# Ugness/MeBT

Measured on AMD Instinct MI355X. Metric: masked video tokens/sec/GPU (train step, 24L d=1024, 1024+256 tok), higher is better.
Workload: dtype bf16; 1 GPU; Sky-Timelapse 16f MeBT train step: 24L/1024d/16h, 1024 VQ tokens + 256 latents, batch 6/GPU, t=0.5 (NC=NT=512), fwd + masked CE + bwd + AdamW; global_batch=6, parallelism=dp1, optimizer=in-backward (fused into the weight-gradient launches)

## Files before the change

### include/mebt_hip.h

```cpp
#ifndef MEBT_HIP_H
#define MEBT_HIP_H

#include <stdint.h>

#ifdef __cplusplus
extern "C" {
#endif

#define MEBT_ABI_VERSION 2
#define MEBT_MAX_LAYERS 128

typedef void* mebt_stream_t;
typedef struct mebt_model mebt_model;

enum mebt_status { MEBT_STATUS_OK = 0, MEBT_STATUS_EINVAL = 1, MEBT_STATUS_ESHAPE = 2, MEBT_STATUS_EHIP = 3,
                   MEBT_STATUS_EWORKSPACE = 4, MEBT_STATUS_EDTYPE = 5 };
enum mebt_dtype { MEBT_DTYPE_F32 = 0, MEBT_DTYPE_BF16 = 1, MEBT_DTYPE_F16 = 2  };
enum mebt_mode { MEBT_MODE_LATENT_ENC = 0, MEBT_MODE_LATENT_SELF = 1, MEBT_MODE_LATENT_DEC = 2, MEBT_MODE_LT2L = 3,
                 MEBT_MODE_MASKGIT = 4  };

typedef struct mebt_model_desc {
    int32_t n_layer, n_head, n_embd, vocab, n_latent , block_size;
    int32_t dtype;
    int32_t modes[MEBT_MAX_LAYERS];
// ... 146 lines not shown
int mebt_op_i3d_head(int32_t dtype, const void* x, const float* w, const float* bias, float* pooled, float* logits, int32_t B, int32_t T,
                     int32_t H, int32_t W, int32_t C, int32_t ncls, mebt_stream_t stream);

int mebt_profile_enable(int32_t on);
int mebt_profile_read(int32_t family, double* launches, double* total_ms, double* total_flops);
int64_t mebt_profile_dump(char* buf, int64_t cap);
int32_t mebt_profile_read_waits(int32_t cap, int32_t* layer, double* ms);
int mebt_debug_dropout_mask(uint64_t seed, uint32_t site, float p, int64_t n, float* out, mebt_stream_t stream);
int mebt_debug_clock_probe(unsigned long long* out4, uint64_t ref_ticks_100mhz, mebt_stream_t stream);
void mebt_debug_side_stream(mebt_model* m, int32_t on);
void mebt_debug_set_side_stream(mebt_model* m, mebt_stream_t stream);
void mebt_debug_gemm_tile(int32_t bm, int32_t bn);
void mebt_debug_gemm_variant(int32_t dma);
void mebt_debug_gemm_scratch(void* buf, int64_t bytes);
void mebt_debug_gemm_stamps(unsigned long long* buf);
void mebt_debug_grouped_config(int32_t tbm, int32_t tbn, int32_t ring);
void mebt_debug_grouped_stages(int32_t n);

#ifdef __cplusplus
}
#endif
#endif
```

### mebt_amd/_lib.py

```python
import ctypes as C
import os

_HERE = os.path.dirname(os.path.abspath(__file__))
LIB_PATH = os.environ.get("MEBT_HIP_LIB") or os.path.join(_HERE, "lib", "libmebt_hip.so")

SHIPPED_TUNE = os.path.join(_HERE, "tune", "gfx950.txt")

MEBT_MAX_LAYERS = 128
F32, BF16, F16 = 0, 1, 2
EPI_NONE, EPI_GELU, EPI_RESID, EPI_GELU_BWD = 0, 1, 2, 3
MODE_IDS = {"latent_enc": 0, "latent_self": 1, "latent_dec": 2, "lt2l": 3, "maskgit": 4}

c_i32, c_i64, c_f32, c_vp = C.c_int32, C.c_int64, C.c_float, C.c_void_p


class ModelDesc(C.Structure):
    _fields_ = [("n_layer", c_i32), ("n_head", c_i32), ("n_embd", c_i32), ("vocab", c_i32),
                ("n_latent", c_i32), ("block_size", c_i32), ("dtype", c_i32),
                ("modes", c_i32 * MEBT_MAX_LAYERS), ("label_smoothing", c_f32),
                ("embd_pdrop", c_f32), ("resid_pdrop", c_f32), ("attn_pdrop", c_f32)]


PROTOTYPES = {
    "mebt_last_error": (C.c_char_p, []),
# ... 48 lines not shown
    "mebt_op_cast_f16": (c_i32, [c_vp, c_vp, c_i64, c_vp]),
    "mebt_op_i3d_preprocess": (c_i32, [c_i32, c_vp, c_vp, c_i32, c_i32, c_i32, c_i32, c_i32, c_vp]),
    "mebt_op_i3d_conv": (c_i32, [c_i32, c_vp, c_vp]),
    "mebt_op_i3d_maxpool": (c_i32, [c_i32, c_vp, c_vp] + [c_i32] * 11 + [c_vp]),
    "mebt_op_i3d_head": (c_i32, [c_i32, c_vp, c_vp, c_vp, c_vp, c_vp] + [c_i32] * 6 + [c_vp]),
    "mebt_debug_dropout_mask": (c_i32, [C.c_uint64, C.c_uint32, c_f32, c_i64, c_vp, c_vp]),
    "mebt_debug_clock_probe": (c_i32, [c_vp, C.c_uint64, c_vp]),
    "mebt_debug_side_stream": (None, [c_vp, c_i32]),
    "mebt_debug_set_side_stream": (None, [c_vp, c_vp]),
    "mebt_debug_gemm_tile": (None, [c_i32, c_i32]),
    "mebt_debug_gemm_variant": (None, [c_i32]),
    "mebt_debug_grouped_stages": (None, [c_i32]),
    "mebt_debug_gemm_scratch": (None, [c_vp, c_i64]),
    "mebt_debug_gemm_stamps": (None, [c_vp]),
    "mebt_debug_grouped_config": (None, [c_i32, c_i32, c_i32]),
    "mebt_gemm_autotune": (None, [c_i32]),
    "mebt_gemm_autotune_enabled": (c_i32, []),
    "mebt_gemm_tune_export": (c_i64, [C.c_char_p, c_i64]),
    "mebt_gemm_tune_import": (c_i32, [C.c_char_p, c_i32]),
    "mebt_gemm_tune_alternatives": (c_i64, [C.c_char_p, c_i64]),
    "mebt_profile_enable": (c_i32, [c_i32]),
    "mebt_profile_read": (c_i32, [c_i32, C.POINTER(C.c_double), C.POINTER(C.c_double), C.POINTER(C.c_double)]),
    "mebt_profile_dump": (c_i64, [C.c_char_p, c_i64]),
    "mebt_profile_read_waits": (c_i32, [c_i32, C.POINTER(C.c_int32), C.POINTER(C.c_double)]),
}

_lib = None


def load():
# ... 53 lines not shown
```

### mebt_amd/csrc/attention.hip

```cpp
#include "common.h"
#include "kernels.h"

namespace {

constexpr int KT = 32;

template <typename T, int HD>
__device__ __forceinline__ void load_row(const T* src, float (&dst)[HD], float scale = 1.f) {
#pragma unroll
    for (int e = 0; e < HD; e += 4) {
        const f32x4 v = load4<T>(src + e);
        dst[e] = v[0] * scale; dst[e + 1] = v[1] * scale; dst[e + 2] = v[2] * scale; dst[e + 3] = v[3] * scale;
    }
}
template <typename T, int HD>
__device__ __forceinline__ void store_row(T* dst, const float (&src)[HD], float scale = 1.f) {
#pragma unroll
    for (int e = 0; e < HD; e += 4) store4<T>(dst + e, f32x4{src[e] * scale, src[e + 1] * scale, src[e + 2] * scale, src[e + 3] * scale});
}

template <typename T, int HD>
__device__ __forceinline__ void stage_tile(float (*dst)[HD], const T* src, int ld, int n, int tid, int nthreads) {
    constexpr int CPR = HD / 4;
    for (int c = tid; c < KT * CPR; c += nthreads) {
// ... 261 lines not shown
        const dim3 gk((p.NK + 63) / 64, p.H, p.B);
        if (NS > 1 && !one && p.NQ >= NS * KT) hipLaunchKernelGGL((attn_bwd_dkv_generic<T, HD, NS>), gk, dim3(64 * NS), (attn_lds_bytes<HD, NS>()), stream, p);
        else hipLaunchKernelGGL((attn_bwd_dkv_generic<T, HD, 1>), gk, dim3(64), (attn_lds_bytes<HD, 1>()), stream, p);
    }
    return MEBT_OK;
}

}

#ifdef MEBT_HAVE_ATTN_MFMA
int launch_attn_fwd_mfma(const AttnParams& p, hipStream_t stream);
int launch_attn_bwd_mfma(const AttnParams& p, hipStream_t stream);
#else
static int launch_attn_fwd_mfma(const AttnParams&, hipStream_t) { return -1; }
static int launch_attn_bwd_mfma(const AttnParams&, hipStream_t) { return -1; }
#endif
#ifdef MEBT_HAVE_ATTN_MFMA
static int g_force_generic = 0;
#else
static int g_force_generic = 1;
#endif
#ifdef MEBT_HAVE_ATTN_MFMA
void mebt_attn_force_generic(int on) { g_force_generic = on; }
#else
void mebt_attn_force_generic(int) {}
#endif

#define DISPATCH_HD(FN, T)                                             \
    switch (p.HD) {                                                    \
        case 32: FN<T, 32>(p, stream); break;                          \
        case 64: FN<T, 64>(p, stream); break;                          \
        case 128: FN<T, 128>(p, stream); break;                        \
        default: mebt_set_error("attention: head size must be 32, 64 or 128"); return MEBT_ESHAPE; \
    }

bool attn_fwd_can_gather(int dtype, int HD) { return dtype == MEBT_BF16 && HD == 64 && !g_force_generic; }

int launch_attn_fwd(const AttnParams& p, int dtype, hipStream_t stream) {
    if (p.B <= 0 || p.NQ <= 0) return MEBT_OK;
    if (dtype == MEBT_BF16 && p.HD == 64 && !g_force_generic && p.NK > 0) return launch_attn_fwd_mfma(p, stream);
    if (p.kidx && p.NK > 0) { mebt_set_error("attention: gathered keys / values (kidx) need the MFMA forward (bf16, head size 64)"); return MEBT_ESHAPE; }
    if (dtype == MEBT_BF16) { DISPATCH_HD(run_fwd, bf16_t) } else { DISPATCH_HD(run_fwd, float) }
// ... 12 lines not shown
```

### mebt_amd/csrc/attention_mfma.hip

```cpp
#include "common.h"
#include "kernels.h"
#include <cstdlib>

namespace {

typedef __attribute__((address_space(3))) s16x4* lds_s16x4_ptr;
typedef short s16x8 __attribute__((ext_vector_type(8)));

constexpr int TILE = 64;
constexpr int TILE_BYTES = TILE * 64 * 2;
constexpr float LOG2E = 1.4426950408889634f;

__device__ __forceinline__ int swz(int row) { return ((row >> 1) & 3) << 1; }

__device__ __forceinline__ bf16x8 frag_rows(const char* tile, int blk16, int ks, int lane) {
    const int row = blk16 * 16 + (lane & 15);
    const int c = 4 * ks + (lane >> 4);
    return *reinterpret_cast<const bf16x8*>(tile + row * 128 + ((c ^ swz(row)) << 4));
}
__device__ __forceinline__ bf16x8 frag_cols(const char* tile, int cb, int kk, int lane) {
    const int g = lane >> 4, i = lane & 15, q4 = i >> 2, pp = i & 3;
    const int ch = 2 * cb + (pp >> 1);
    const int r0 = 32 * kk + 4 * g + q4, r1 = r0 + 16;
    const s16x4 lo = __builtin_amdgcn_ds_read_tr16_b64_v4i16((lds_s16x4_ptr)(tile + r0 * 128 + ((ch ^ swz(r0)) << 4) + 8 * (pp & 1)));
// ... 46 lines not shown
}
typedef unsigned u32x2_t __attribute__((ext_vector_type(2)));
__device__ __forceinline__ float group_sum(float v) {
    u32x2_t r = __builtin_amdgcn_permlane16_swap(__float_as_uint(v), __float_as_uint(v), false, false);
    v = __uint_as_float(r[0]) + __uint_as_float(r[1]);
    r = __builtin_amdgcn_permlane32_swap(__float_as_uint(v), __float_as_uint(v), false, false);
    return __uint_as_float(r[0]) + __uint_as_float(r[1]);
}
__device__ __forceinline__ float group_max(float v) {
    u32x2_t r = __builtin_amdgcn_permlane16_swap(__float_as_uint(v), __float_as_uint(v), false, false);
    v = fmaxf(__uint_as_float(r[0]), __uint_as_float(r[1]));
    r = __builtin_amdgcn_permlane32_swap(__float_as_uint(v), __float_as_uint(v), false, false);
    return fmaxf(__uint_as_float(r[0]), __uint_as_float(r[1]));
}
#define MFMA(a, b, c) __builtin_amdgcn_mfma_f32_16x16x32_bf16(a, b, c, 0, 0, 0)

constexpr int WAVES = 8;
constexpr int BLOCK_ROWS = WAVES * 16;
constexpr int CHUNK_TILES = 4;
constexpr int CHUNK = CHUNK_TILES * TILE;
constexpr int CHUNK_BYTES = CHUNK_TILES * TILE_BYTES;
constexpr int STAT_BYTES = CHUNK * 4;
constexpr int MASK_BYTES = 4096;
constexpr int MASK_OFF = 2 * CHUNK_BYTES + 2 * STAT_BYTES;
constexpr int STAGE_BYTES = MASK_OFF + MASK_BYTES;
constexpr int ATTN_LDS = 2 * STAGE_BYTES;
constexpr int DMA_PER_WAVE = 2 * (CHUNK_BYTES / 1024) / WAVES;

template <int NW = WAVES>
struct ChunkDma {
// ... 26 lines not shown
            const uint32_t off = src[i] >= 0 ? ((uint32_t)src[i] * ld + 8 * (slot ^ swz(row))) * 2 : (uint32_t)MEBT_OOB;
            dma16(rsrc, lds_addr_of(dst + (wave + NW * i) * 1024), off);
        }
    }
};
template <int N> __device__ __forceinline__ void wait_vm() { asm volatile("s_waitcnt vmcnt(%0)" ::"n"(N) : "memory"); }

template <int NW, int NST, int SPLIT = 1>
__global__ __launch_bounds__(NW * SPLIT * 64) void attn_fwd_mfma(const AttnParams p) {
    extern __shared__ __attribute__((aligned(16))) char smem_all[];
    constexpr int CT = NW / 2, CROWS = CT * TILE, CBYTES = CT * TILE_BYTES, SBYTES = 2 * CBYTES;
    const int tid = threadIdx.x, lane = tid & 63, g = lane >> 4;
    const int wave_all = __builtin_amdgcn_readfirstlane(tid >> 6);
    const int half = SPLIT == 1 ? 0 : wave_all / NW, wave = SPLIT == 1 ? wave_all : wave_all % NW;
    char* smem = smem_all + half * (NST * SBYTES);
    const int b = blockIdx.z, h = blockIdx.y;
    const int q = blockIdx.x * (NW * 16) + wave * 16 + (lane & 15);
    const bf16_t* Q = reinterpret_cast<const bf16_t*>(p.q) + (size_t)b * p.NQ * p.ldq + h * 64;
    const bool gather = p.kidx != nullptr;
    const int krows = gather ? p.kidx_rows : p.NK;
    const bf16_t* K = reinterpret_cast<const bf16_t*>(p.k) + (size_t)b * krows * p.ldk + h * 64;
    const bf16_t* V = reinterpret_cast<const bf16_t*>(p.v) + (size_t)b * krows * p.ldv + h * 64;
    bf16x8 qf[2];
#pragma unroll
    for (int ks = 0; ks < 2; ++ks) qf[ks] = frag_global(Q, q, p.NQ, p.ldq, ks, lane);
    ChunkDma<NW> lk, lv;
    lk.init(K, krows, p.ldk, wave, lane);
    lv.init(V, krows, p.ldv, wave, lane);
    int* sidx = reinterpret_cast<int*>(smem_all + SPLIT * NST * SBYTES);
    if (gather) {
        const int32_t* gi = p.kidx + (size_t)b * p.NK;
        for (int i = tid; i < p.NK; i += NW * SPLIT * 64) sidx[i] = gi[i];
// ... 148 lines not shown
        const float inv = 1.0f / l;
        bf16_t* O = reinterpret_cast<bf16_t*>(p.o) + ((size_t)b * p.NQ + q) * p.ldo + h * 64;
#pragma unroll
        for (int e = 0; e < 4; ++e) store4<bf16_t>(O + 16 * e + 4 * g, o[e] * inv);
        if (p.lse && g == 0) p.lse[((size_t)b * p.H + h) * p.NQ + q] = m * 0.6931471805599453f + logf(l);
    }
}

__global__ __launch_bounds__(512) void attn_fwd_pp(const AttnParams p) {
    extern __shared__ __attribute__((aligned(16))) char smem_all[];
    constexpr int NW = 4, CROWS = 2 * TILE, CBYTES = 2 * TILE_BYTES, SBYTES = 2 * CBYTES;
    const int tid = threadIdx.x, lane = tid & 63, g = lane >> 4;
    const int wave_all = __builtin_amdgcn_readfirstlane(tid >> 6);
    const int half = wave_all >> 2, wave = wave_all & 3;
    char* smem = smem_all + half * (2 * SBYTES);
    const int b = blockIdx.z, h = blockIdx.y;
    const int q = blockIdx.x * (NW * 16) + wave * 16 + (lane & 15);
    const bf16_t* Q = reinterpret_cast<const bf16_t*>(p.q) + (size_t)b * p.NQ * p.ldq + h * 64;
    const bool gather = p.kidx != nullptr;
    const int krows = gather ? p.kidx_rows : p.NK;
    const bf16_t* K = reinterpret_cast<const bf16_t*>(p.k) + (size_t)b * krows * p.ldk + h * 64;
    const bf16_t* V = reinterpret_cast<const bf16_t*>(p.v) + (size_t)b * krows * p.ldv + h * 64;
    bf16x8 qf[2];
#pragma unroll
    for (int ks = 0; ks < 2; ++ks) qf[ks] = frag_global(Q, q, p.NQ, p.ldq, ks, lane);
    ChunkDma<NW> lk, lv;
    lk.init(K, krows, p.ldk, wave, lane);
    lv.init(V, krows, p.ldv, wave, lane);
    int* sidx = reinterpret_cast<int*>(smem_all + 4 * SBYTES);
    if (gather) {
        const int32_t* gi = p.kidx + (size_t)b * p.NK;
        for (int i = tid; i < p.NK; i += 512) sidx[i] = gi[i];
// ... 154 lines not shown
#pragma unroll
        for (int e = 0; e < 4; ++e)
#pragma unroll
            for (int rr = 0; rr < 4; ++rr) o[e][rr] = o[e][rr] * a0 + mg[4 * e + rr] * a1;
        m = mn;
    }
    if (q < p.NQ) {
        const float inv = 1.0f / l;
        bf16_t* O = reinterpret_cast<bf16_t*>(p.o) + ((size_t)b * p.NQ + q) * p.ldo + h * 64;
#pragma unroll
        for (int e = 0; e < 4; ++e) store4<bf16_t>(O + 16 * e + 4 * g, o[e] * inv);
        if (p.lse && g == 0) p.lse[((size_t)b * p.H + h) * p.NQ + q] = m * 0.6931471805599453f + logf(l);
    }
}

__global__ __launch_bounds__(WAVES * 64) void attn_bwd_dq_mfma(const AttnParams p) {
    extern __shared__ __attribute__((aligned(16))) char smem[];
    const int tid = threadIdx.x, lane = tid & 63, g = lane >> 4;
    const int wave = __builtin_amdgcn_readfirstlane(tid >> 6);
    const int b = blockIdx.z, h = blockIdx.y;
    const int q = blockIdx.x * BLOCK_ROWS + wave * 16 + (lane & 15);
    const bool qv = q < p.NQ;
    const bf16_t* Q = reinterpret_cast<const bf16_t*>(p.q) + (size_t)b * p.NQ * p.ldq + h * 64;
    const bf16_t* G = reinterpret_cast<const bf16_t*>(p.d_o) + (size_t)b * p.NQ * p.lddo + h * 64;
    const bf16_t* Oo = reinterpret_cast<const bf16_t*>(p.o) + (size_t)b * p.NQ * p.ldo + h * 64;
    const bf16_t* K = reinterpret_cast<const bf16_t*>(p.k) + (size_t)b * p.NK * p.ldk + h * 64;
    const bf16_t* V = reinterpret_cast<const bf16_t*>(p.v) + (size_t)b * p.NK * p.ldv + h * 64;
    ChunkDma<> lk, lv;
    lk.init(K, p.NK, p.ldk, wave, lane);
    lv.init(V, p.NK, p.ldv, wave, lane);
    const int nchunks = (p.NK + CHUNK - 1) / CHUNK;
    bf16x8 qf[2], gf[2], of[2];
#pragma unroll
    for (int ks = 0; ks < 2; ++ks) {
        qf[ks] = frag_global(Q, q, p.NQ, p.ldq, ks, lane);
        gf[ks] = frag_global(G, q, p.NQ, p.lddo, ks, lane);
        of[ks] = frag_global(Oo, q, p.NQ, p.ldo, ks, lane);
    }
    const size_t sidx = ((size_t)b * p.H + h) * p.NQ + q;
    const float lse_q = qv ? p.lse[sidx] : 0.f;
    const bool use_bits = p.drop.thresh && p.dmask != nullptr;
    const int mtiles = mebt_attn_dmask_tiles(p.NK);
    const size_t mrow0 = ((size_t)b * p.H + h) * p.NQ;
    const __amdgpu_buffer_rsrc_t rmask = make_rsrc(p.dmask ? p.dmask + mrow0 * mtiles * 4 : (const uint16_t*)p.q, use_bits ? (size_t)p.NQ * mtiles * 8 : 0);
    const uint32_t moff = (uint32_t)((blockIdx.x * BLOCK_ROWS + 32 * (wave & 3) + (lane >> 1)) * mtiles * 8 + (lane & 1) * 16);
    auto issue_mask = [&](char* stage, int chunk) {
        if (wave < 4) dma16(rmask, lds_addr_of(stage + MASK_OFF + wave * 1024), moff + (uint32_t)chunk * 32);
    };
    lk.issue(smem, 0, wave);
    lv.issue(smem + CHUNK_BYTES, 0, wave);
    issue_mask(smem, 0);
    if (nchunks > 1) {
        lk.issue(smem + STAGE_BYTES, 1, wave);
        lv.issue(smem + STAGE_BYTES + CHUNK_BYTES, 1, wave);
        issue_mask(smem + STAGE_BYTES, 1);
    }
    float delta = 0.f;
#pragma unroll
    for (int ks = 0; ks < 2; ++ks)
#pragma unroll
        for (int j = 0; j < 8; ++j) delta += (float)gf[ks][j] * (float)of[ks][j];
    delta = group_sum(delta);
    const float lse2 = lse_q * LOG2E;
    const float c = 0.125f * LOG2E;
    FragOffsets fo;
    fo.init(lane);

    f32x4 dq[4];
#pragma unroll
    for (int e = 0; e < 4; ++e) dq[e] = f32x4{0, 0, 0, 0};
    const uint64_t drow = (((uint64_t)b * p.H + h) * p.NQ + q) * p.NK;
    const int mlds = (wave * 16 + (lane & 15)) * 32 + g * 2;
    for (int ch = 0; ch < nchunks; ++ch) {
        char* stage = smem + (ch & 1) * STAGE_BYTES;
        if (ch + 1 < nchunks) { if (wave < 4) wait_vm<DMA_PER_WAVE + 1>(); else wait_vm<DMA_PER_WAVE>(); } else wait_vm<0>();
        __builtin_amdgcn_s_barrier();
        const int nt = min(CHUNK_TILES, (p.NK - ch * CHUNK + TILE - 1) / TILE);
// ... 40 lines not shown
        if (ch + 2 < nchunks) {
            __builtin_amdgcn_s_barrier();
            lk.issue(stage, ch + 2, wave);
            lv.issue(stage + CHUNK_BYTES, ch + 2, wave);
            issue_mask(stage, ch + 2);
        }
    }
    if (qv) {
        bf16_t* D = reinterpret_cast<bf16_t*>(p.dq) + ((size_t)b * p.NQ + q) * p.lddq + h * 64;
#pragma unroll
        for (int e = 0; e < 4; ++e) store4<bf16_t>(D + 16 * e + 4 * g, dq[e]);
        if (g == 0) p.delta[sidx] = delta;
    }
}

__global__ __launch_bounds__(WAVES * 64) void attn_bwd_dkv_mfma(const AttnParams p) {
    extern __shared__ __attribute__((aligned(16))) char smem[];
    const int tid = threadIdx.x, lane = tid & 63, g = lane >> 4;
    const int wave = __builtin_amdgcn_readfirstlane(tid >> 6);
    const int b = blockIdx.z, h = blockIdx.y;
    const int key = blockIdx.x * BLOCK_ROWS + wave * 16 + (lane & 15);
    const bf16_t* Q = reinterpret_cast<const bf16_t*>(p.q) + (size_t)b * p.NQ * p.ldq + h * 64;
    const bf16_t* G = reinterpret_cast<const bf16_t*>(p.d_o) + (size_t)b * p.NQ * p.lddo + h * 64;
    const bf16_t* K = reinterpret_cast<const bf16_t*>(p.k) + (size_t)b * p.NK * p.ldk + h * 64;
    const bf16_t* V = reinterpret_cast<const bf16_t*>(p.v) + (size_t)b * p.NK * p.ldv + h * 64;
    const float* L = p.lse + ((size_t)b * p.H + h) * p.NQ;
    const float* Dl = p.delta + ((size_t)b * p.H + h) * p.NQ;
    ChunkDma<> lq, lg;
    lq.init(Q, p.NQ, p.ldq, wave, lane);
    lg.init(G, p.NQ, p.lddo, wave, lane);
    const __amdgpu_buffer_rsrc_t rstat = make_rsrc(wave == 0 ? L : Dl, (size_t)p.NQ * 4);
    const int nchunks = (p.NQ + CHUNK - 1) / CHUNK;
    const bool use_bits = p.drop.thresh && p.dmask != nullptr;
    const int mtiles = mebt_attn_dmask_tiles(p.NK);
    const size_t mrow0 = ((size_t)b * p.H + h) * p.NQ;
    const __amdgpu_buffer_rsrc_t rmask = make_rsrc(p.dmask ? p.dmask + mrow0 * mtiles * 4 : (const uint16_t*)p.q, use_bits ? (size_t)p.NQ * mtiles * 8 : 0);
    const uint32_t moff = (uint32_t)((64 * (wave & 3) + lane) * mtiles * 8 + blockIdx.x * 16);
    auto issue = [&](char* stage, int chunk) {
        lq.issue(stage, chunk, wave);
        lg.issue(stage + CHUNK_BYTES, chunk, wave);
        if (wave < 2) dma16(rstat, lds_addr_of(stage + 2 * CHUNK_BYTES + wave * STAT_BYTES), (uint32_t)(chunk * CHUNK * 4 + lane * 16));
        if (wave < 4) dma16(rmask, lds_addr_of(stage + MASK_OFF + wave * 1024), moff + (uint32_t)chunk * CHUNK * (uint32_t)mtiles * 8);
    };
    bf16x8 kf[2], vf[2];
#pragma unroll
    for (int ks = 0; ks < 2; ++ks) {
        kf[ks] = frag_global(K, key, p.NK, p.ldk, ks, lane);
        vf[ks] = frag_global(V, key, p.NK, p.ldv, ks, lane);
    }
    issue(smem, 0);
    if (nchunks > 1) issue(smem + STAGE_BYTES, 1);
    const float c = 0.125f * LOG2E;
    FragOffsets fo;
    fo.init(lane);

    f32x4 dk[4], dv[4];
#pragma unroll
    for (int e = 0; e < 4; ++e) { dk[e] = f32x4{0, 0, 0, 0}; dv[e] = f32x4{0, 0, 0, 0}; }
    const uint64_t dcol = ((uint64_t)b * p.H + h) * p.NQ * p.NK + key;
    for (int ch = 0; ch < nchunks; ++ch) {
        char* stage = smem + (ch & 1) * STAGE_BYTES;
        if (ch + 1 < nchunks) {
            if (wave < 2) wait_vm<DMA_PER_WAVE + 2>(); else if (wave < 4) wait_vm<DMA_PER_WAVE + 1>(); else wait_vm<DMA_PER_WAVE>();
        } else {
            wait_vm<0>();
        }
        __builtin_amdgcn_s_barrier();
        const float* cl = reinterpret_cast<const float*>(stage + 2 * CHUNK_BYTES);
        const float* cd = cl + CHUNK;
        const char* cm = stage + MASK_OFF + (wave >> 2) * 8 + ((lane >> 2) & 3) * 2;
        const int mbit = 4 * (wave & 3) + (lane & 3);
        const int nt = min(CHUNK_TILES, (p.NQ - ch * CHUNK + TILE - 1) / TILE);
        for (int t = 0; t < nt; t += 2) {
            f32x4 pr[2][4], ds[2][4];
#pragma unroll
            for (int u = 0; u < 2; ++u) {
                const char* sQ = stage + (t + u) * TILE_BYTES;
                const char* sG = stage + CHUNK_BYTES + (t + u) * TILE_BYTES;
// ... 23 lines not shown
#pragma unroll
            for (int u = 0; u < 2; ++u)
#pragma unroll
                for (int kk = 0; kk < 2; ++kk) {
                    const bf16x8 pf = pack_acc(pr[u][2 * kk], pr[u][2 * kk + 1]);
                    const bf16x8 df = pack_acc(ds[u][2 * kk], ds[u][2 * kk + 1]);
#pragma unroll
                    for (int e = 0; e < 4; ++e) {
                        dv[e] = MFMA(fo.col_frag(stage + CHUNK_BYTES + (t + u) * TILE_BYTES, e, kk), pf, dv[e]);
                        dk[e] = MFMA(fo.col_frag(stage + (t + u) * TILE_BYTES, e, kk), df, dk[e]);
                    }
                }
        }
        if (ch + 2 < nchunks) {
            __builtin_amdgcn_s_barrier();
            issue(stage, ch + 2);
        }
    }
    if (key < p.NK) {
        bf16_t* DK = reinterpret_cast<bf16_t*>(p.dk) + ((size_t)b * p.NK + key) * p.lddk + h * 64;
        bf16_t* DV = reinterpret_cast<bf16_t*>(p.dv) + ((size_t)b * p.NK + key) * p.lddv + h * 64;
#pragma unroll
        for (int e = 0; e < 4; ++e) {
            store4<bf16_t>(DK + 16 * e + 4 * g, dk[e]);
            store4<bf16_t>(DV + 16 * e + 4 * g, dv[e]);
        }
    }
}

}

static int check_layout(const AttnParams& p) {
    if (p.HD != 64) { mebt_set_error("mfma attention: head size must be 64"); return MEBT_ESHAPE; }
    if ((p.ldq | p.ldk | p.ldv | p.ldo) % 8) { mebt_set_error("mfma attention: row strides must be multiples of 8 elements"); return MEBT_ESHAPE; }
    static bool inited = false;
    if (!inited) {
        MEBT_HIP_CHECK(hipFuncSetAttribute(reinterpret_cast<const void*>(&attn_fwd_mfma<8, 2>), hipFuncAttributeMaxDynamicSharedMemorySize, 160 * 1024));
        MEBT_HIP_CHECK(hipFuncSetAttribute(reinterpret_cast<const void*>(&attn_fwd_mfma<8, 1>), hipFuncAttributeMaxDynamicSharedMemorySize, 160 * 1024));
        MEBT_HIP_CHECK(hipFuncSetAttribute(reinterpret_cast<const void*>(&attn_fwd_mfma<4, 2>), hipFuncAttributeMaxDynamicSharedMemorySize, 160 * 1024));
        MEBT_HIP_CHECK(hipFuncSetAttribute(reinterpret_cast<const void*>(&attn_fwd_mfma<4, 4>), hipFuncAttributeMaxDynamicSharedMemorySize, 160 * 1024));
        MEBT_HIP_CHECK(hipFuncSetAttribute(reinterpret_cast<const void*>(&attn_fwd_mfma<4, 2, 2>), hipFuncAttributeMaxDynamicSharedMemorySize, 160 * 1024));
        MEBT_HIP_CHECK(hipFuncSetAttribute(reinterpret_cast<const void*>(&attn_fwd_pp), hipFuncAttributeMaxDynamicSharedMemorySize, 160 * 1024));
        MEBT_HIP_CHECK(hipFuncSetAttribute(reinterpret_cast<const void*>(&attn_bwd_dq_mfma), hipFuncAttributeMaxDynamicSharedMemorySize, ATTN_LDS));
        MEBT_HIP_CHECK(hipFuncSetAttribute(reinterpret_cast<const void*>(&attn_bwd_dkv_mfma), hipFuncAttributeMaxDynamicSharedMemorySize, ATTN_LDS));
        inited = true;
    }
    return MEBT_OK;
}
static int lds_bytes(int streamed_rows) { return streamed_rows <= CHUNK ? STAGE_BYTES : ATTN_LDS; }

int launch_attn_fwd_mfma(const AttnParams& p_in, hipStream_t stream) {
    AttnParams p = p_in;
    drop_mark_small(p.drop, (uint64_t)p.B * p.H * p.NQ * p.NK);
    if (int rc = check_layout(p)) return rc;
    static const int force = [] { const char* e = getenv("MEBT_ATTN_FWD_WAVES"); return e ? atoi(e) : 0; }();
    const long grid8 = (long)((p.NQ + 127) / 128) * p.H * p.B;
    const bool four = force ? force == 4 : grid8 <= 128;
    const int xl = p.kidx ? ((p.NK * 4 + 15) & ~15) : 0;
    if (xl && xl + 4 * CHUNK_BYTES > 160 * 1024) { mebt_set_error("mfma attention: a gathered key set holds at most 8192 keys"); return MEBT_ESHAPE; }
    if (four) {
        const dim3 grid((p.NQ + 63) / 64, p.H, p.B);
        static const int split_on = [] { const char* e = getenv("MEBT_ATTN_FWD_SPLIT"); return e ? atoi(e) : 1; }();
        if (p.NK <= 1024) hipLaunchKernelGGL((attn_fwd_mfma<4, 2>), grid, dim3(256), 2 * CHUNK_BYTES + xl, stream, p);
        else if (split_on && (long)grid.x * p.H * p.B <= 256) {
            if (split_on == 2) hipLaunchKernelGGL((attn_fwd_mfma<4, 2, 2>), grid, dim3(512), 4 * CHUNK_BYTES + xl, stream, p);
            else hipLaunchKernelGGL(attn_fwd_pp, grid, dim3(512), 4 * CHUNK_BYTES + xl, stream, p);
        }
        else hipLaunchKernelGGL((attn_fwd_mfma<4, 4>), grid, dim3(256), 4 * CHUNK_BYTES + xl, stream, p);
    } else {
        const dim3 grid((p.NQ + BLOCK_ROWS - 1) / BLOCK_ROWS, p.H, p.B);
        if (p.NK <= CHUNK) hipLaunchKernelGGL((attn_fwd_mfma<8, 1>), grid, dim3(WAVES * 64), 2 * CHUNK_BYTES + xl, stream, p);
        else hipLaunchKernelGGL((attn_fwd_mfma<8, 2>), grid, dim3(WAVES * 64), 2 * 2 * CHUNK_BYTES + xl, stream, p);
    }
    MEBT_HIP_CHECK(hipGetLastError());
    return MEBT_OK;
}

int launch_attn_bwd_mfma(const AttnParams& p_in, hipStream_t stream) {
    AttnParams p = p_in;
    drop_mark_small(p.drop, (uint64_t)p.B * p.H * p.NQ * p.NK);
    if (int rc = check_layout(p)) return rc;
    if ((p.lddo | p.lddq | p.lddk | p.lddv) % 8) { mebt_set_error("mfma attention: row strides must be multiples of 8 elements"); return MEBT_ESHAPE; }
    const dim3 gq((p.NQ + BLOCK_ROWS - 1) / BLOCK_ROWS, p.H, p.B);
    hipLaunchKernelGGL(attn_bwd_dq_mfma, gq, dim3(WAVES * 64), lds_bytes(p.NK), stream, p);
    const dim3 gk((p.NK + BLOCK_ROWS - 1) / BLOCK_ROWS, p.H, p.B);
    hipLaunchKernelGGL(attn_bwd_dkv_mfma, gk, dim3(WAVES * 64), lds_bytes(p.NQ), stream, p);
    MEBT_HIP_CHECK(hipGetLastError());
    return MEBT_OK;
}
```

### mebt_amd/csrc/capi.cpp

```cpp
#include "common.h"
#include "kernels.h"
#include <cmath>
#include "../../include/mebt_hip.h"
#include <string.h>

static hipStream_t S(mebt_stream_t s) { return reinterpret_cast<hipStream_t>(s); }
static int check_dtype(int dtype) {
    if (dtype == MEBT_F32 || dtype == MEBT_BF16) return MEBT_OK;
    mebt_set_error("unsupported dtype (0 = f32, 1 = bf16)");
    return MEBT_EDTYPE;
}

extern "C" int mebt_op_gemm(int32_t dtype, const void* A, const void* B, void* C, void* C2, const float* bias, const void* aux,
                            int32_t M, int32_t N, int32_t K, int32_t lda, int32_t ldb, int32_t ldc, int32_t ld_aux,
                            int32_t a_kc, int32_t b_kc, int32_t epilogue, int32_t c_f32, int32_t beta, int32_t split_k,
                            mebt_stream_t stream) {
    if (int rc = check_dtype(dtype)) return rc;
    if (!A || !B || (!C && epilogue != EPI_GELU)) { mebt_set_error("gemm: null operand"); return MEBT_EINVAL; }
    if (epilogue < EPI_NONE || epilogue > EPI_GELU_BWD) { mebt_set_error("gemm: bad epilogue"); return MEBT_EINVAL; }
    if ((epilogue == EPI_RESID || epilogue == EPI_GELU_BWD) && !aux) { mebt_set_error("gemm: epilogue needs aux"); return MEBT_EINVAL; }
    if (epilogue == EPI_GELU && !C2) { mebt_set_error("gemm: GELU epilogue needs C2"); return MEBT_EINVAL; }
    if (M < 0 || N < 0 || K <= 0) { mebt_set_error("gemm: bad extents"); return MEBT_ESHAPE; }
    static bool inited = false;
    if (!inited) { if (int rc = gemm_init_attributes()) return rc; inited = true; }
// ... 38 lines not shown
    p.seg = 0; p.seg_stride = 0; p.seg_off = 0;
    return launch_ln_fwd(p, dtype, S(stream));
}

extern "C" int mebt_op_layernorm_bwd(int32_t dtype, const void* x, const void* dy, const float* gamma, const float* mean,
                                     const float* rstd, void* dx, float* dgamma, float* dbeta, int32_t rows, int32_t d,
                                     mebt_stream_t stream) {
    if (int rc = check_dtype(dtype)) return rc;
    if (!x || !dy || !gamma || !mean || !rstd || !dx || !dgamma || !dbeta) { mebt_set_error("layernorm_bwd: null pointer"); return MEBT_EINVAL; }
    LnBwdParams p;
    p.x = x; p.dy = dy; p.dy2 = nullptr; p.dx_add = nullptr; p.gamma = gamma; p.mean = mean; p.rstd = rstd; p.dx = dx; p.dx_f32 = dtype == MEBT_F32;
    p.dx_accumulate = 0; p.dgamma = dgamma; p.dbeta = dbeta; p.rows = rows; p.d = d; p.seg = 0; p.seg_stride = 0; p.seg_off = 0;
    return launch_ln_bwd(p, dtype, S(stream));
}

extern "C" int mebt_op_attention_fwd(int32_t dtype, const void* q, const void* k, const void* v, void* o, float* lse, int32_t B,
                                     int32_t H, int32_t NQ, int32_t NK, int32_t HD, int32_t ldq, int32_t ldk, int32_t ldv,
                                     int32_t ldo, int32_t force_generic, mebt_stream_t stream) {
    if (int rc = check_dtype(dtype)) return rc;
    if (!q || !o || (NK > 0 && (!k || !v))) { mebt_set_error("attention: null pointer"); return MEBT_EINVAL; }
    AttnParams p;
    memset(&p, 0, sizeof(p));
    p.q = q; p.k = k; p.v = v; p.o = o; p.lse = lse; p.B = B; p.H = H; p.NQ = NQ; p.NK = NK; p.HD = HD;
    p.ldq = ldq; p.ldk = ldk; p.ldv = ldv; p.ldo = ldo;
    mebt_attn_force_generic(force_generic);
    const int rc = launch_attn_fwd(p, dtype, S(stream));
    mebt_attn_force_generic(0);
    return rc;
}

extern "C" int mebt_op_attention_bwd(int32_t dtype, const void* q, const void* k, const void* v, const void* o, const float* lse,
                                     const void* d_o, void* dq, void* dk, void* dv, float* delta, int32_t B, int32_t H,
                                     int32_t NQ, int32_t NK, int32_t HD, int32_t ldq, int32_t ldk, int32_t ldv, int32_t ldo,
                                     int32_t force_generic, mebt_stream_t stream) {
    if (int rc = check_dtype(dtype)) return rc;
    if (!q || !o || !lse || !d_o || !dq || !delta || (NK > 0 && (!k || !v || !dk || !dv))) { mebt_set_error("attention_bwd: null pointer"); return MEBT_EINVAL; }
    AttnParams p;
    memset(&p, 0, sizeof(p));
    p.q = q; p.k = k; p.v = v; p.o = const_cast<void*>(o); p.lse = const_cast<float*>(lse); p.B = B; p.H = H; p.NQ = NQ; p.NK = NK; p.HD = HD;
    p.ldq = ldq; p.ldk = ldk; p.ldv = ldv; p.ldo = ldo;
    p.d_o = d_o; p.dq = dq; p.dk = dk; p.dv = dv; p.delta = delta; p.lddo = ldo; p.lddq = ldq; p.lddk = ldk; p.lddv = ldv;
    mebt_attn_force_generic(force_generic);
    const int rc = launch_attn_bwd(p, dtype, S(stream));
    mebt_attn_force_generic(0);
    return rc;
}

extern "C" int mebt_op_embed_fwd(int32_t dtype, const int64_t* x_ids, const int64_t* ci, const int64_t* ti, const float* tok_emb,
                                 const float* pos_emb, const float* mask_emb, const float* sos_emb, void* sos, void* ctx, void* tgt,
                                 int32_t B, int32_t N, int32_t NC, int32_t NT, int32_t NS, int32_t d, int32_t vocab,
                                 int32_t block_size, mebt_stream_t stream) {
    if (int rc = check_dtype(dtype)) return rc;
    if (!x_ids || !tok_emb || !pos_emb || !mask_emb) { mebt_set_error("embed: null pointer"); return MEBT_EINVAL; }
    if (N > block_size) { mebt_set_error("embed: N exceeds block_size"); return MEBT_ESHAPE; }
    EmbedParams p;
    p.x_ids = x_ids; p.ci = ci; p.ti = ti; p.tok_emb = tok_emb; p.pos_emb = pos_emb; p.mask_emb = mask_emb; p.sos_emb = sos_emb;
// ... 78 lines not shown
```

### mebt_amd/csrc/kernels.h

```cpp
#pragma once
#include <hip/hip_runtime.h>
#include <stdint.h>
#include <cstdlib>
#include "common.h"

enum { MEBT_F32 = 0, MEBT_BF16 = 1 };
enum { SITE_ATTN = 0, SITE_PROJ = 1, SITE_MLP = 2, SITE_EMB_SOS = 0xFFFF0, SITE_EMB_CTX = 0xFFFF1, SITE_EMB_TGT = 0xFFFF2 };
static inline DropCfg make_drop(uint64_t seed, uint32_t site, float p) {
    DropCfg d;
    d.seed = seed; d.site = site;
    d.thresh = p > 0.f ? (uint32_t)((double)p * 65536.0 + 0.5) : 0u;
    d.inv_keep = d.thresh ? (float)(65536.0 / (65536.0 - d.thresh)) : 1.0f;
    d.small = 0;
    d.base32 = site * 0x632BE5ABu + (uint32_t)(seed >> 32);
    return d;
}
static inline void drop_mark_small(DropCfg& d, uint64_t n_elems) {
    static const bool on = [] { const char* e = getenv("MEBT_DROP_SMALL"); return !(e && e[0] == '0'); }();
    d.small = (on && n_elems < (1ull << 33)) ? 1u : 0u;
}
enum { EPI_NONE = 0, EPI_GELU = 1, EPI_RESID = 2, EPI_GELU_BWD = 3, EPI_ADAMW = 4  };

struct GemmScratch { void* flush; size_t flush_bytes; float* splitk; size_t splitk_bytes; };
#define MEBT_TUNE_FLUSH_BYTES (384ull << 20)
// ... 145 lines not shown
    int g_bf16 = 0;
    int g_pieces = 1;
    size_t g_stride = 0;
};
int launch_adamw(const AdamWParams& p, hipStream_t stream);
int launch_cast_f32_to_bf16(const float* src, void* dst, size_t n, hipStream_t stream);

struct AttnParams {
    const void* q; const void* k; const void* v; void* o; float* lse;
    int B, H, NQ, NK, HD; int ldq, ldk, ldv, ldo;
    const void* d_o; void* dq; void* dk; void* dv; float* delta; int lddo, lddq, lddk, lddv;
    DropCfg drop;
    uint16_t* dmask = nullptr;
    const int32_t* kidx = nullptr;
    int kidx_rows = 0;
};
__host__ __device__ static inline int mebt_attn_dmask_tiles(int NK) { return 4 * ((NK + 255) / 256); }
static inline size_t mebt_attn_dmask_bytes(int B, int H, int NQ, int NK) { return (size_t)B * H * NQ * mebt_attn_dmask_tiles(NK) * 8; }
int launch_attn_fwd(const AttnParams& p, int dtype, hipStream_t stream);
int launch_attn_bwd(const AttnParams& p, int dtype, hipStream_t stream);
void mebt_attn_force_generic(int on);
bool attn_fwd_can_gather(int dtype, int HD);

struct SampleParams {
    const float* logits;
    int logits_bf16 = 0;
    int icdf = 0;
    const float* noise;
    uint64_t noise_seed = 0;
    float temperature; int top_k; float top_p;
    int64_t* ids;
    float* score;
    float* probs;
    int rows, V;
    float* kth = nullptr;
    const int64_t* probs_ti = nullptr;
// ... 12 lines not shown
```

Before: 314,500 masked tokens/s (whole job).

## Fuse attention backward into one launch with XCD-aware block ordering and in-kernel delta

Flattens attention grids to 1D and remaps block indices so consecutive (batch, head) tiles land on the same XCD, aiming to improve L2 reuse of K/V across chiplets. Merges the dQ and dK/dV backward kernels into a single launch, so the two halves can overlap instead of running back to back. The dK/dV half now computes the per-row delta from dO and O itself, removing its dependency on the delta written by the dQ half. The cost is extra global loads and LDS stores per chunk, plus a larger shared-memory footprint, which may lower occupancy. Legacy paths stay selectable through an env var or debug bit, and debug hooks for attention dropout and block order are added.

```diff
diff --git a/include/mebt_hip.h b/include/mebt_hip.h
--- a/include/mebt_hip.h
+++ b/include/mebt_hip.h
@@ -184,6 +184,9 @@
 void mebt_debug_gemm_variant(int32_t dma);
 void mebt_debug_gemm_scratch(void* buf, int64_t bytes);
 void mebt_debug_gemm_stamps(unsigned long long* buf);
+void mebt_debug_attn_dropout(uint64_t seed, float p, void* dmask);
+void mebt_debug_attn_legacy(int32_t bits);
+int mebt_debug_attn_block_order(int32_t T, int32_t X, int32_t H, int32_t xcd, int32_t* pos_to_id, mebt_stream_t stream);
 void mebt_debug_grouped_config(int32_t tbm, int32_t tbn, int32_t ring);
 void mebt_debug_grouped_stages(int32_t n);
 
diff --git a/mebt_amd/_lib.py b/mebt_amd/_lib.py
--- a/mebt_amd/_lib.py
+++ b/mebt_amd/_lib.py
@@ -86,6 +86,9 @@
     "mebt_debug_gemm_scratch": (None, [c_vp, c_i64]),
     "mebt_debug_gemm_stamps": (None, [c_vp]),
     "mebt_debug_grouped_config": (None, [c_i32, c_i32, c_i32]),
+    "mebt_debug_attn_dropout": (None, [C.c_uint64, c_f32, c_vp]),
+    "mebt_debug_attn_legacy": (None, [c_i32]),
+    "mebt_debug_attn_block_order": (c_i32, [c_i32, c_i32, c_i32, c_i32, c_vp, c_vp]),
     "mebt_gemm_autotune": (None, [c_i32]),
     "mebt_gemm_autotune_enabled": (c_i32, []),
     "mebt_gemm_tune_export": (c_i64, [C.c_char_p, c_i64]),
diff --git a/mebt_amd/csrc/attention.hip b/mebt_amd/csrc/attention.hip
--- a/mebt_amd/csrc/attention.hip
+++ b/mebt_amd/csrc/attention.hip
@@ -299,6 +299,7 @@
 #else
 static int launch_attn_fwd_mfma(const AttnParams&, hipStream_t) { return -1; }
 static int launch_attn_bwd_mfma(const AttnParams&, hipStream_t) { return -1; }
+int launch_attn_block_order_probe(int, int, int, int, int32_t*, hipStream_t) { mebt_set_error("built without the MFMA attention"); return MEBT_EINVAL; }
 #endif
 #ifdef MEBT_HAVE_ATTN_MFMA
 static int g_force_generic = 0;
@@ -311,6 +312,13 @@
 void mebt_attn_force_generic(int) {}
 #endif
 
+static int g_attn_legacy = -1;
+void mebt_attn_set_legacy(int bits) { g_attn_legacy = bits; }
+int mebt_attn_legacy() {
+    static const int env = [] { const char* e = getenv("MEBT_ATTN_LEGACY"); return e ? atoi(e) : 0; }();
+    return g_attn_legacy >= 0 ? g_attn_legacy : env;
+}
+
 #define DISPATCH_HD(FN, T)                                             \
     switch (p.HD) {                                                    \
         case 32: FN<T, 32>(p, stream); break;                          \
diff --git a/mebt_amd/csrc/attention_mfma.hip b/mebt_amd/csrc/attention_mfma.hip
--- a/mebt_amd/csrc/attention_mfma.hip
+++ b/mebt_amd/csrc/attention_mfma.hip
@@ -84,6 +84,29 @@
     return fmaxf(__uint_as_float(r[0]), __uint_as_float(r[1]));
 }
 #define MFMA(a, b, c) __builtin_amdgcn_mfma_f32_16x16x32_bf16(a, b, c, 0, 0, 0)
+
+struct BlockPos { int x, h, b; };
+__device__ __forceinline__ BlockPos attn_block_pos(int t, int T, int X, int H, bool xcd) {
+    int j = t;
+    if (xcd) {
+        const int q = T >> 3, r = T & 7, c = t & 7;
+        j = c * q + min(c, r) + (t >> 3);
+    }
+    BlockPos bp;
+    bp.x = j % X;
+    const int hb = j / X;
+    bp.h = hb % H;
+    bp.b = hb / H;
+    return bp;
+}
+__device__ __forceinline__ float row_delta(const bf16x8 (&gf)[2], const bf16x8 (&of)[2]) {
+    float delta = 0.f;
+#pragma unroll
+    for (int ks = 0; ks < 2; ++ks)
+#pragma unroll
+        for (int j = 0; j < 8; ++j) delta += (float)gf[ks][j] * (float)of[ks][j];
+    return group_sum(delta);
+}
 
 constexpr int WAVES = 8;
 constexpr int BLOCK_ROWS = WAVES * 16;
@@ -140,8 +163,9 @@
     const int wave_all = __builtin_amdgcn_readfirstlane(tid >> 6);
     const int half = SPLIT == 1 ? 0 : wave_all / NW, wave = SPLIT == 1 ? wave_all : wave_all % NW;
     char* smem = smem_all + half * (NST * SBYTES);
-    const int b = blockIdx.z, h = blockIdx.y;
-    const int q = blockIdx.x * (NW * 16) + wave * 16 + (lane & 15);
+    const BlockPos bp = attn_block_pos(blockIdx.x, gridDim.x, (p.NQ + NW * 16 - 1) / (NW * 16), p.H, p.xcd_order);
+    const int b = bp.b, h = bp.h;
+    const int q = bp.x * (NW * 16) + wave * 16 + (lane & 15);
     const bf16_t* Q = reinterpret_cast<const bf16_t*>(p.q) + (size_t)b * p.NQ * p.ldq + h * 64;
     const bool gather = p.kidx != nullptr;
     const int krows = gather ? p.kidx_rows : p.NK;
@@ -320,8 +344,9 @@
     const int wave_all = __builtin_amdgcn_readfirstlane(tid >> 6);
     const int half = wave_all >> 2, wave = wave_all & 3;
     char* smem = smem_all + half * (2 * SBYTES);
-    const int b = blockIdx.z, h = blockIdx.y;
-    const int q = blockIdx.x * (NW * 16) + wave * 16 + (lane & 15);
+    const BlockPos bp = attn_block_pos(blockIdx.x, gridDim.x, (p.NQ + NW * 16 - 1) / (NW * 16), p.H, p.xcd_order);
+    const int b = bp.b, h = bp.h;
+    const int q = bp.x * (NW * 16) + wave * 16 + (lane & 15);
     const bf16_t* Q = reinterpret_cast<const bf16_t*>(p.q) + (size_t)b * p.NQ * p.ldq + h * 64;
     const bool gather = p.kidx != nullptr;
     const int krows = gather ? p.kidx_rows : p.NK;
@@ -506,12 +531,10 @@
     }
 }
 
-__global__ __launch_bounds__(WAVES * 64) void attn_bwd_dq_mfma(const AttnParams p) {
-    extern __shared__ __attribute__((aligned(16))) char smem[];
+__device__ __forceinline__ void bwd_dq_block(const AttnParams& p, char* smem, int xb, int h, int b) {
     const int tid = threadIdx.x, lane = tid & 63, g = lane >> 4;
     const int wave = __builtin_amdgcn_readfirstlane(tid >> 6);
-    const int b = blockIdx.z, h = blockIdx.y;
-    const int q = blockIdx.x * BLOCK_ROWS + wave * 16 + (lane & 15);
+    const int q = xb * BLOCK_ROWS + wave * 16 + (lane & 15);
     const bool qv = q < p.NQ;
     const bf16_t* Q = reinterpret_cast<const bf16_t*>(p.q) + (size_t)b * p.NQ * p.ldq + h * 64;
     const bf16_t* G = reinterpret_cast<const bf16_t*>(p.d_o) + (size_t)b * p.NQ * p.lddo + h * 64;
@@ -535,7 +558,7 @@
     const int mtiles = mebt_attn_dmask_tiles(p.NK);
     const size_t mrow0 = ((size_t)b * p.H + h) * p.NQ;
     const __amdgpu_buffer_rsrc_t rmask = make_rsrc(p.dmask ? p.dmask + mrow0 * mtiles * 4 : (const uint16_t*)p.q, use_bits ? (size_t)p.NQ * mtiles * 8 : 0);
-    const uint32_t moff = (uint32_t)((blockIdx.x * BLOCK_ROWS + 32 * (wave & 3) + (lane >> 1)) * mtiles * 8 + (lane & 1) * 16);
+    const uint32_t moff = (uint32_t)((xb * BLOCK_ROWS + 32 * (wave & 3) + (lane >> 1)) * mtiles * 8 + (lane & 1) * 16);
     auto issue_mask = [&](char* stage, int chunk) {
         if (wave < 4) dma16(rmask, lds_addr_of(stage + MASK_OFF + wave * 1024), moff + (uint32_t)chunk * 32);
     };
@@ -547,12 +570,7 @@
         lv.issue(smem + STAGE_BYTES + CHUNK_BYTES, 1, wave);
         issue_mask(smem + STAGE_BYTES, 1);
     }
-    float delta = 0.f;
-#pragma unroll
-    for (int ks = 0; ks < 2; ++ks)
-#pragma unroll
-        for (int j = 0; j < 8; ++j) delta += (float)gf[ks][j] * (float)of[ks][j];
-    delta = group_sum(delta);
+    const float delta = row_delta(gf, of);
     const float lse2 = lse_q * LOG2E;
     const float c = 0.125f * LOG2E;
     FragOffsets fo;
@@ -623,14 +641,14 @@
     }
 }
 
-__global__ __launch_bounds__(WAVES * 64) void attn_bwd_dkv_mfma(const AttnParams p) {
-    extern __shared__ __attribute__((aligned(16))) char smem[];
+template <bool OWN_DELTA>
+__device__ __forceinline__ void bwd_dkv_block(const AttnParams& p, char* smem, int xb, int h, int b) {
     const int tid = threadIdx.x, lane = tid & 63, g = lane >> 4;
     const int wave = __builtin_amdgcn_readfirstlane(tid >> 6);
-    const int b = blockIdx.z, h = blockIdx.y;
-    const int key = blockIdx.x * BLOCK_ROWS + wave * 16 + (lane & 15);
+    const int key = xb * BLOCK_ROWS + wave * 16 + (lane & 15);
     const bf16_t* Q = reinterpret_cast<const bf16_t*>(p.q) + (size_t)b * p.NQ * p.ldq + h * 64;
     const bf16_t* G = reinterpret_cast<const bf16_t*>(p.d_o) + (size_t)b * p.NQ * p.lddo + h * 64;
+    const bf16_t* Oo = reinterpret_cast<const bf16_t*>(p.o) + (size_t)b * p.NQ * p.ldo + h * 64;
     const bf16_t* K = reinterpret_cast<const bf16_t*>(p.k) + (size_t)b * p.NK * p.ldk + h * 64;
     const bf16_t* V = reinterpret_cast<const bf16_t*>(p.v) + (size_t)b * p.NK * p.ldv + h * 64;
     const float* L = p.lse + ((size_t)b * p.H + h) * p.NQ;
@@ -638,17 +656,18 @@
     ChunkDma<> lq, lg;
     lq.init(Q, p.NQ, p.ldq, wave, lane);
     lg.init(G, p.NQ, p.lddo, wave, lane);
+    constexpr int NSTAT = OWN_DELTA ? 1 : 2;
     const __amdgpu_buffer_rsrc_t rstat = make_rsrc(wave == 0 ? L : Dl, (size_t)p.NQ * 4);
     const int nchunks = (p.NQ + CHUNK - 1) / CHUNK;
     const bool use_bits = p.drop.thresh && p.dmask != nullptr;
     const int mtiles = mebt_attn_dmask_tiles(p.NK);
     const size_t mrow0 = ((size_t)b * p.H + h) * p.NQ;
     const __amdgpu_buffer_rsrc_t rmask = make_rsrc(p.dmask ? p.dmask + mrow0 * mtiles * 4 : (const uint16_t*)p.q, use_bits ? (size_t)p.NQ * mtiles * 8 : 0);
-    const uint32_t moff = (uint32_t)((64 * (wave & 3) + lane) * mtiles * 8 + blockIdx.x * 16);
+    const uint32_t moff = (uint32_t)((64 * (wave & 3) + lane) * mtiles * 8 + xb * 16);
     auto issue = [&](char* stage, int chunk) {
         lq.issue(stage, chunk, wave);
         lg.issue(stage + CHUNK_BYTES, chunk, wave);
-        if (wave < 2) dma16(rstat, lds_addr_of(stage + 2 * CHUNK_BYTES + wave * STAT_BYTES), (uint32_t)(chunk * CHUNK * 4 + lane * 16));
+        if (wave < NSTAT) dma16(rstat, lds_addr_of(stage + 2 * CHUNK_BYTES + wave * STAT_BYTES), (uint32_t)(chunk * CHUNK * 4 + lane * 16));
         if (wave < 4) dma16(rmask, lds_addr_of(stage + MASK_OFF + wave * 1024), moff + (uint32_t)chunk * CHUNK * (uint32_t)mtiles * 8);
     };
     bf16x8 kf[2], vf[2];
@@ -657,8 +676,37 @@
         kf[ks] = frag_global(K, key, p.NK, p.ldk, ks, lane);
         vf[ks] = frag_global(V, key, p.NK, p.ldv, ks, lane);
     }
-    issue(smem, 0);
-    if (nchunks > 1) issue(smem + STAGE_BYTES, 1);
+    auto load_delta_rows = [&](bf16x8 (&df)[2][2][2], int chunk) {
+#pragma unroll
+        for (int j = 0; j < 2; ++j)
+#pragma unroll
+            for (int ks = 0; ks < 2; ++ks) {
+                const int row = chunk * CHUNK + 32 * wave + 16 * j + (lane & 15);
+                df[j][0][ks] = frag_global(G, row, p.NQ, p.lddo, ks, lane);
+                df[j][1][ks] = frag_global(Oo, row, p.NQ, p.ldo, ks, lane);
+            }
+    };
+    auto store_delta = [&](const bf16x8 (&df)[2][2][2], char* stage) {
+        float* cd = reinterpret_cast<float*>(stage + 2 * CHUNK_BYTES + STAT_BYTES);
+#pragma unroll
+        for (int j = 0; j < 2; ++j) {
+            const float d = row_delta(df[j][0], df[j][1]);
+            if (g == 0) cd[32 * wave + 16 * j + (lane & 15)] = d;
+        }
+    };
+    if (OWN_DELTA) {
+        bf16x8 d0[2][2][2], d1[2][2][2];
+        load_delta_rows(d0, 0);
+        if (nchunks > 1) load_delta_rows(d1, 1);
+        issue(smem, 0);
+        if (nchunks > 1) issue(smem + STAGE_BYTES, 1);
+        store_delta(d0, smem);
+        if (nchunks > 1) store_delta(d1, smem + STAGE_BYTES);
+        asm volatile("s_waitcnt lgkmcnt(0)" ::: "memory");
+    } else {
+        issue(smem, 0);
+        if (nchunks > 1) issue(smem + STAGE_BYTES, 1);
+    }
     const float c = 0.125f * LOG2E;
     FragOffsets fo;
     fo.init(lane);
@@ -670,7 +718,7 @@
     for (int ch = 0; ch < nchunks; ++ch) {
         char* stage = smem + (ch & 1) * STAGE_BYTES;
         if (ch + 1 < nchunks) {
-            if (wave < 2) wait_vm<DMA_PER_WAVE + 2>(); else if (wave < 4) wait_vm<DMA_PER_WAVE + 1>(); else wait_vm<DMA_PER_WAVE>();
+            if (wave < NSTAT) wait_vm<DMA_PER_WAVE + 2>(); else if (wave < 4) wait_vm<DMA_PER_WAVE + 1>(); else wait_vm<DMA_PER_WAVE>();
         } else {
             wait_vm<0>();
         }
@@ -724,7 +772,15 @@
         }
         if (ch + 2 < nchunks) {
             __builtin_amdgcn_s_barrier();
-            issue(stage, ch + 2);
+            if (OWN_DELTA) {
+                bf16x8 d2[2][2][2];
+                load_delta_rows(d2, ch + 2);
+                issue(stage, ch + 2);
+                store_delta(d2, stage);
+                asm volatile("s_waitcnt lgkmcnt(0)" ::: "memory");
+            } else {
+                issue(stage, ch + 2);
+            }
         }
     }
     if (key < p.NK) {
@@ -738,6 +794,43 @@
     }
 }
 
+__global__ __launch_bounds__(WAVES * 64) void attn_bwd_dq_mfma(const AttnParams p) {
+    extern __shared__ __attribute__((aligned(16))) char smem[];
+    const BlockPos bp = attn_block_pos(blockIdx.x, gridDim.x, (p.NQ + BLOCK_ROWS - 1) / BLOCK_ROWS, p.H, p.xcd_order);
+    bwd_dq_block(p, smem, bp.x, bp.h, bp.b);
+}
+__global__ __launch_bounds__(WAVES * 64) void attn_bwd_dkv_mfma(const AttnParams p) {
+    extern __shared__ __attribute__((aligned(16))) char smem[];
+    const BlockPos bp = attn_block_pos(blockIdx.x, gridDim.x, (p.NK + BLOCK_ROWS - 1) / BLOCK_ROWS, p.H, p.xcd_order);
+    bwd_dkv_block<false>(p, smem, bp.x, bp.h, bp.b);
+}
+__global__ __launch_bounds__(WAVES * 64) void attn_bwd_mfma(const AttnParams p) {
+    extern __shared__ __attribute__((aligned(16))) char smem[];
+    const int xk = (p.NK + BLOCK_ROWS - 1) / BLOCK_ROWS, tk = xk * p.H * p.B;
+    const int t = blockIdx.x;
+    if (t < tk) {
+        const BlockPos bp = attn_block_pos(t, tk, xk, p.H, p.xcd_order);
+        bwd_dkv_block<true>(p, smem, bp.x, bp.h, bp.b);
+    } else {
+        const BlockPos bp = attn_block_pos(t - tk, gridDim.x - tk, (p.NQ + BLOCK_ROWS - 1) / BLOCK_ROWS, p.H, p.xcd_order);
+        bwd_dq_block(p, smem, bp.x, bp.h, bp.b);
+    }
+}
+
+__global__ void attn_block_order_probe(int T, int X, int H, int xcd, int32_t* pos_to_id) {
+    if (threadIdx.x) return;
+    const BlockPos bp = attn_block_pos(blockIdx.x, T, X, H, xcd);
+    if (bp.x < 0 || bp.x >= X || bp.h < 0 || bp.h >= H || bp.b < 0 || bp.b >= T / (X * H)) return;
+    pos_to_id[((size_t)bp.b * H + bp.h) * X + bp.x] = (int32_t)blockIdx.x;
+}
+
+}
+
+int launch_attn_block_order_probe(int T, int X, int H, int xcd, int32_t* pos_to_id, hipStream_t stream) {
+    if (T <= 0 || X <= 0 || H <= 0 || T % (X * H)) { mebt_set_error("attention block order: T must be a positive multiple of X * H"); return MEBT_ESHAPE; }
+    hipLaunchKernelGGL(attn_block_order_probe, dim3(T), dim3(64), 0, stream, T, X, H, xcd, pos_to_id);
+    MEBT_HIP_CHECK(hipGetLastError());
+    return MEBT_OK;
 }
 
 static int check_layout(const AttnParams& p) {
@@ -753,6 +846,7 @@
         MEBT_HIP_CHECK(hipFuncSetAttribute(reinterpret_cast<const void*>(&attn_fwd_pp), hipFuncAttributeMaxDynamicSharedMemorySize, 160 * 1024));
         MEBT_HIP_CHECK(hipFuncSetAttribute(reinterpret_cast<const void*>(&attn_bwd_dq_mfma), hipFuncAttributeMaxDynamicSharedMemorySize, ATTN_LDS));
         MEBT_HIP_CHECK(hipFuncSetAttribute(reinterpret_cast<const void*>(&attn_bwd_dkv_mfma), hipFuncAttributeMaxDynamicSharedMemorySize, ATTN_LDS));
+        MEBT_HIP_CHECK(hipFuncSetAttribute(reinterpret_cast<const void*>(&attn_bwd_mfma), hipFuncAttributeMaxDynamicSharedMemorySize, ATTN_LDS));
         inited = true;
     }
     return MEBT_OK;
@@ -763,22 +857,23 @@
     AttnParams p = p_in;
     drop_mark_small(p.drop, (uint64_t)p.B * p.H * p.NQ * p.NK);
     if (int rc = check_layout(p)) return rc;
+    p.xcd_order = !(mebt_attn_legacy() & 1);
     static const int force = [] { const char* e = getenv("MEBT_ATTN_FWD_WAVES"); return e ? atoi(e) : 0; }();
     const long grid8 = (long)((p.NQ + 127) / 128) * p.H * p.B;
     const bool four = force ? force == 4 : grid8 <= 128;
     const int xl = p.kidx ? ((p.NK * 4 + 15) & ~15) : 0;
     if (xl && xl + 4 * CHUNK_BYTES > 160 * 1024) { mebt_set_error("mfma attention: a gathered key set holds at most 8192 keys"); return MEBT_ESHAPE; }
     if (four) {
-        const dim3 grid((p.NQ + 63) / 64, p.H, p.B);
+        const dim3 grid((p.NQ + 63) / 64 * p.H * p.B);
         static const int split_on = [] { const char* e = getenv("MEBT_ATTN_FWD_SPLIT"); return e ? atoi(e) : 1; }();
         if (p.NK <= 1024) hipLaunchKernelGGL((attn_fwd_mfma<4, 2>), grid, dim3(256), 2 * CHUNK_BYTES + xl, stream, p);
-        else if (split_on && (long)grid.x * p.H * p.B <= 256) {
+        else if (split_on && (long)grid.x <= 256) {
             if (split_on == 2) hipLaunchKernelGGL((attn_fwd_mfma<4, 2, 2>), grid, dim3(512), 4 * CHUNK_BYTES + xl, stream, p);
             else hipLaunchKernelGGL(attn_fwd_pp, grid, dim3(512), 4 * CHUNK_BYTES + xl, stream, p);
         }
         else hipLaunchKernelGGL((attn_fwd_mfma<4, 4>), grid, dim3(256), 4 * CHUNK_BYTES + xl, stream, p);
     } else {
-        const dim3 grid((p.NQ + BLOCK_ROWS - 1) / BLOCK_ROWS, p.H, p.B);
+        const dim3 grid((p.NQ + BLOCK_ROWS - 1) / BLOCK_ROWS * p.H * p.B);
         if (p.NK <= CHUNK) hipLaunchKernelGGL((attn_fwd_mfma<8, 1>), grid, dim3(WAVES * 64), 2 * CHUNK_BYTES + xl, stream, p);
         else hipLaunchKernelGGL((attn_fwd_mfma<8, 2>), grid, dim3(WAVES * 64), 2 * 2 * CHUNK_BYTES + xl, stream, p);
     }
@@ -791,10 +886,15 @@
     drop_mark_small(p.drop, (uint64_t)p.B * p.H * p.NQ * p.NK);
     if (int rc = check_layout(p)) return rc;
     if ((p.lddo | p.lddq | p.lddk | p.lddv) % 8) { mebt_set_error("mfma attention: row strides must be multiples of 8 elements"); return MEBT_ESHAPE; }
-    const dim3 gq((p.NQ + BLOCK_ROWS - 1) / BLOCK_ROWS, p.H, p.B);
-    hipLaunchKernelGGL(attn_bwd_dq_mfma, gq, dim3(WAVES * 64), lds_bytes(p.NK), stream, p);
-    const dim3 gk((p.NK + BLOCK_ROWS - 1) / BLOCK_ROWS, p.H, p.B);
-    hipLaunchKernelGGL(attn_bwd_dkv_mfma, gk, dim3(WAVES * 64), lds_bytes(p.NQ), stream, p);
+    const int legacy = mebt_attn_legacy();
+    p.xcd_order = !(legacy & 1);
+    const int tq = (p.NQ + BLOCK_ROWS - 1) / BLOCK_ROWS * p.H * p.B, tk = (p.NK + BLOCK_ROWS - 1) / BLOCK_ROWS * p.H * p.B;
+    if (legacy & 2) {
+        hipLaunchKernelGGL(attn_bwd_dq_mfma, dim3(tq), dim3(WAVES * 64), lds_bytes(p.NK), stream, p);
+        hipLaunchKernelGGL(attn_bwd_dkv_mfma, dim3(tk), dim3(WAVES * 64), lds_bytes(p.NQ), stream, p);
+    } else {
+        hipLaunchKernelGGL(attn_bwd_mfma, dim3(tk + tq), dim3(WAVES * 64), max(lds_bytes(p.NK), lds_bytes(p.NQ)), stream, p);
+    }
     MEBT_HIP_CHECK(hipGetLastError());
     return MEBT_OK;
 }
diff --git a/mebt_amd/csrc/capi.cpp b/mebt_amd/csrc/capi.cpp
--- a/mebt_amd/csrc/capi.cpp
+++ b/mebt_amd/csrc/capi.cpp
@@ -76,6 +76,18 @@
     return launch_ln_bwd(p, dtype, S(stream));
 }
 
+static DropCfg g_op_attn_drop = make_drop(0, 0, 0.f);
+static uint16_t* g_op_attn_dmask = nullptr;
+extern "C" void mebt_debug_attn_dropout(uint64_t seed, float p, void* dmask) {
+    g_op_attn_drop = make_drop(seed, SITE_ATTN, p);
+    g_op_attn_dmask = p > 0.f ? (uint16_t*)dmask : nullptr;
+}
+extern "C" void mebt_debug_attn_legacy(int32_t bits) { mebt_attn_set_legacy(bits); }
+extern "C" int mebt_debug_attn_block_order(int32_t T, int32_t X, int32_t H, int32_t xcd, int32_t* pos_to_id, mebt_stream_t stream) {
+    if (!pos_to_id) { mebt_set_error("attention block order: null pointer"); return MEBT_EINVAL; }
+    return launch_attn_block_order_probe(T, X, H, xcd, pos_to_id, S(stream));
+}
+
 extern "C" int mebt_op_attention_fwd(int32_t dtype, const void* q, const void* k, const void* v, void* o, float* lse, int32_t B,
                                      int32_t H, int32_t NQ, int32_t NK, int32_t HD, int32_t ldq, int32_t ldk, int32_t ldv,
                                      int32_t ldo, int32_t force_generic, mebt_stream_t stream) {
@@ -85,6 +97,7 @@
     memset(&p, 0, sizeof(p));
     p.q = q; p.k = k; p.v = v; p.o = o; p.lse = lse; p.B = B; p.H = H; p.NQ = NQ; p.NK = NK; p.HD = HD;
     p.ldq = ldq; p.ldk = ldk; p.ldv = ldv; p.ldo = ldo;
+    p.drop = g_op_attn_drop; p.dmask = g_op_attn_dmask;
     mebt_attn_force_generic(force_generic);
     const int rc = launch_attn_fwd(p, dtype, S(stream));
     mebt_attn_force_generic(0);
@@ -102,6 +115,7 @@
     p.q = q; p.k = k; p.v = v; p.o = const_cast<void*>(o); p.lse = const_cast<float*>(lse); p.B = B; p.H = H; p.NQ = NQ; p.NK = NK; p.HD = HD;
     p.ldq = ldq; p.ldk = ldk; p.ldv = ldv; p.ldo = ldo;
     p.d_o = d_o; p.dq = dq; p.dk = dk; p.dv = dv; p.delta = delta; p.lddo = ldo; p.lddq = ldq; p.lddk = ldk; p.lddv = ldv;
+    p.drop = g_op_attn_drop; p.dmask = g_op_attn_dmask;
     mebt_attn_force_generic(force_generic);
     const int rc = launch_attn_bwd(p, dtype, S(stream));
     mebt_attn_force_generic(0);
diff --git a/mebt_amd/csrc/kernels.h b/mebt_amd/csrc/kernels.h
--- a/mebt_amd/csrc/kernels.h
+++ b/mebt_amd/csrc/kernels.h
@@ -183,12 +183,16 @@
     uint16_t* dmask = nullptr;
     const int32_t* kidx = nullptr;
     int kidx_rows = 0;
+    int xcd_order = 0;
 };
 __host__ __device__ static inline int mebt_attn_dmask_tiles(int NK) { return 4 * ((NK + 255) / 256); }
 static inline size_t mebt_attn_dmask_bytes(int B, int H, int NQ, int NK) { return (size_t)B * H * NQ * mebt_attn_dmask_tiles(NK) * 8; }
 int launch_attn_fwd(const AttnParams& p, int dtype, hipStream_t stream);
 int launch_attn_bwd(const AttnParams& p, int dtype, hipStream_t stream);
 void mebt_attn_force_generic(int on);
+void mebt_attn_set_legacy(int bits);
+int mebt_attn_legacy();
+int launch_attn_block_order_probe(int T, int X, int H, int xcd, int32_t* pos_to_id, hipStream_t stream);
 bool attn_fwd_can_gather(int dtype, int HD);
 
 struct SampleParams {
```

After: 319,500 masked tokens/s (whole job), median of 6. 1.02x the previous value.
